# meffmadd/intro-tc-vae

Hardware: AMD Instinct MI355X
Metric: images/sec (64x64x3, z=128, bs=64) intro-TC step (higher is better)
Workload: dtype f32 in/out/accumulate, conv products on split-fp16 MFMA (two scaled fp16 planes, 3 products, fp32-class); 1 GPU; c2: IntroTCSovler.train_step, conv arch, 64x64x3, z_dim=128, channels (64, 128, 256, 512), batch 64/GPU, Adam lr 2e-4, clip 100, N=10000; global_batch=64, parallelism=single, sync_bn=False

## Files before the change

include/itcv_hip.h:

```cpp
#ifndef ITCV_HIP_H
#define ITCV_HIP_H

#include <stddef.h>
#include <stdint.h>

#ifdef __cplusplus
extern "C" {
#endif

#define ITCV_ABI_VERSION 4

int itcv_abi_version(void);
const char* itcv_last_error(void);
int itcv_set_option(const char* name, int value);
int itcv_get_option(const char* name);

int itcv_profile_begin(void);
int itcv_profile_end(void);
int itcv_profile_get(int i, int* code, double* flop, float* ms);
int itcv_profile_clear(void);

size_t itcv_conv2d_packed_weight_elems(int Co, int Ci, int KS, int for_dgrad);
int itcv_conv2d_pack_weight(const float* w, float* wp, int Co, int Ci, int KS, int for_dgrad,
                            void* stream);
// ... 62 lines not shown
int itcv_conv2d_small_cin_bf16x3_supported(int C, int Co, int KS, int W);
int itcv_conv2d_small_cin_fwd_bf16x3(const float* x, const float* w, const float* bias, float* y, int B, int C, int H,
                                     int W, int Co, int KS, int for_dgrad, int ns ,
                                     const float* x_amax , void* stream);
int itcv_conv2d_wgrad_bf16s_supported(int Ci, int H, int W, int Co, int KS);
int itcv_conv2d_wgrad_bf16s(const float* x, const float* dy, float* dw, int B, int Ci, int H, int W, int Co,
                            int KS, int ns, int accumulate, void* ws, size_t ws_bytes, void* stream);
size_t itcv_conv2d_wgrad_workspace(int B, int Ci, int H, int W, int Co, int KS);
int itcv_conv2d_wgrad(const float* x, const float* dy, float* dw, int B, int Ci, int H, int W,
                      int Co, int KS, int up2, int accumulate, void* ws, size_t ws_bytes, void* stream);
int itcv_conv2d_fwd_variant(int B, int Ci, int H, int W, int Co, int KS, int up2);
int itcv_conv2d_wgrad_variant(int B, int Ci, int H, int W, int Co, int KS, int up2);
size_t itcv_bias_grad_workspace(int B, int C, int HW);
int itcv_bias_grad(const float* dy, float* db, int B, int C, int HW, int accumulate, void* ws,
                   size_t ws_bytes, void* stream);

size_t itcv_bn_workspace(int B, int C, int HW);
int itcv_bn_moments(const float* x, double* sums, int B, int C, int HW, void* ws, size_t ws_bytes,
                    void* stream);
int itcv_bn_train_stats(const float* x, int B, int C, int HW, float eps, float momentum, float* running_mean,
                        float* running_var, int64_t* num_batches_tracked, float* mean, float* rstd, void* ws,
                        size_t ws_bytes, void* stream);
int itcv_bn_finalize(const double* sums, double count, float eps, float momentum, float* running_mean,
                     float* running_var, int64_t* num_batches_tracked, float* mean, float* rstd, int C,
                     void* stream);
int itcv_bn_finalize_uv(const double* sums, double count, float eps, float momentum, float* running_mean,
                        float* running_var, int64_t* num_batches_tracked, float* mean, float* rstd, float* unbiased_var,
                        int C, void* stream);
int itcv_bn_eval_stats(const float* running_mean, const float* running_var, float eps, float* mean,
                       float* rstd, int C, void* stream);
// ... 192 lines not shown
                        int loss_type, int reduction, float scale, void* stream);
int itcv_exp_elbo_fwd(const float* a, const float* b, float* out, float* w, int B, float c, void* stream);
int itcv_exp_elbo_bwd(const float* g, const float* w, float* da, float* db, int B, void* stream);
int itcv_lincomb_fwd(const float* const* terms, const float* weights, int n, float* out, void* stream);
int itcv_lincomb_bwd(const float* g, const float* weights, int n, float* grads, void* stream);

size_t itcv_sumsq_workspace(size_t n);
int itcv_sumsq(const float* x, size_t n, double* out, void* ws, size_t ws_bytes, void* stream);
int itcv_clip_coef(const double* sumsq, int nparts, double clip, float* norm_out, float* coef_out,
                   void* stream);
int itcv_scale_by_dev(float* x, size_t n, const float* coef_dev, void* stream);
int itcv_adam_step(float* p, const float* g, float* m, float* v, size_t n, float lr, float beta1,
                   float beta2, float eps, int step, void* stream);
int itcv_adam_step_dev(float* p, const float* g, float* m, float* v, size_t n, float lr, float beta1,
                       float beta2, float eps, int* step_dev, void* stream);
#define ITCV_OPT_MAXIMIZE 0x1
#define ITCV_OPT_NESTEROV 0x2
#define ITCV_OPT_AMSGRAD 0x4
#define ITCV_OPT_DECOUPLED_WD 0x8
#define ITCV_OPT_CENTERED 0x10
int itcv_adamx_step_dev(float* p, const float* g, float* exp_avg, float* exp_avg_sq, float* max_exp_avg_sq,
                        const unsigned char* live, size_t n, double lr, double beta1, double beta2, double eps,
                        double weight_decay, int flags, int* step_dev, void* stream);
int itcv_sgd_step_dev(float* p, const float* g, float* momentum_buffer, const unsigned char* live, size_t n, double lr,
                      double momentum, double dampening, double weight_decay, int flags, int* step_dev, void* stream);
int itcv_adagrad_step_dev(float* p, const float* g, float* sum, const unsigned char* live, size_t n, double lr,
                          double lr_decay, double weight_decay, double eps, int flags, int* step_dev, void* stream);
int itcv_rmsprop_step_dev(float* p, const float* g, float* square_avg, float* momentum_buffer, float* grad_avg,
                          const unsigned char* live, size_t n, double lr, double alpha, double eps,
                          double weight_decay, double momentum, int flags, int* step_dev, void* stream);
// ... 10 lines not shown
```

intro-tc-vae_amd/csrc/conv_igemm.hip:

```cpp
#include "conv_shared.h"

namespace itcv {



constexpr uint32_t kOobBase = 0x80000000u;

__device__ __forceinline__ float buf_load_s(__amdgpu_buffer_rsrc_t r, uint32_t voff, uint32_t soff) {
  return __builtin_bit_cast(float, __builtin_amdgcn_raw_buffer_load_b32(r, voff, __builtin_amdgcn_readfirstlane(soff), 0));
}

__host__ __device__ inline int tile_rows_for(int M) { return M <= 32 ? 32 : (M <= 64 ? 64 : 128); }

struct ConvArgs {
  const float* x;
  const float* wp;
  const float* bias;
  float* y;
  int B, Ci, H, W, Co;
  int Cip, Mp, N;
  int mt, nt;
  int ktiles, ktiles_per_split, cpt;
  uint32_t x_bytes;
  size_t slab_stride;
// ... 1876 lines not shown
  const size_t beg = (size_t)s * chunk, end = beg + chunk < total ? beg + chunk : total;
  double acc = 0.0;
  for (size_t i = beg + threadIdx.x; i < end; i += 256) {
    const size_t b = i / HW, hw = i - b * HW;
    acc += (double)dy[(b * C + c) * HW + hw];
  }
  acc = block_sum(acc, scratch);
  if (threadIdx.x == 0) part[(size_t)s * C + c] = acc;
}
__global__ void bias_grad_combine(const double* __restrict__ part, float* __restrict__ db, int C, int splits,
                                  int accumulate) {
  const int c = blockIdx.x * blockDim.x + threadIdx.x;
  if (c >= C) return;
  const double s = fold_strided(0.0, part + c, (size_t)C, splits);
  db[c] = (accumulate ? db[c] : 0.f) + (float)s;
}

static inline int pad_to(int c, int m) { return (c + m - 1) / m * m; }
static inline int pad16(int c) { return pad_to(c, 16); }
static inline int pad32(int c) { return pad_to(c, 32); }

static int check_ws(const char* name, const void* ws, size_t ws_bytes, size_t need) {
  if (need && (!ws || ws_bytes < need)) return fail("%s: workspace too small (need %lld bytes)", name, (long long)need);
  return 0;
}

static int reduce_fwd_splits(const char* name, const void* ws, const float* bias, float* y, size_t out_elems, int splits,
                             int HW, int Co, hipStream_t st) {
  if (splits <= 1) return 0;
  const int blocks = (int)(cdivz(out_elems, 256) < 2048 ? cdivz(out_elems, 256) : 2048);
// ... 869 lines not shown
}

int itcv_bias_grad(const float* dy, float* db, int B, int C, int HW, int accumulate, void* ws, size_t ws_bytes,
                   void* stream) {
  ITCV_REQUIRE(dy && db && B > 0 && C > 0 && HW > 0, "itcv_bias_grad");
  const int splits = bias_splits(B, C, HW);
  ITCV_REQUIRE(ws && ws_bytes >= (size_t)splits * C * sizeof(double), "itcv_bias_grad(workspace)");
  double* part = static_cast<double*>(ws);
  hipLaunchKernelGGL(bias_grad_partial, dim3(C, splits), dim3(256), 0, S(stream), dy, part, B, C, HW, splits);
  ITCV_CHECK_LAUNCH("itcv_bias_grad");
  hipLaunchKernelGGL(bias_grad_combine, dim3(cdiv(C, 256)), dim3(256), 0, S(stream), part, db, C, splits, accumulate);
  ITCV_CHECK_LAUNCH("itcv_bias_grad(combine)");
  return 0;
}

}
```

intro-tc-vae_amd/csrc/loss_optim.hip:

```cpp
#include <math.h>

#include "common.h"

namespace itcv {

template <int LT>
__device__ __forceinline__ float rec_err(float r, float t) {
  if (LT == ITCV_LOSS_MSE) {
    const float d = r - t;
    return d * d;
  }
  if (LT == ITCV_LOSS_L1) return fabsf(r - t);
  return -(t * fmaxf(logf(r), -100.f) + (1.f - t) * fmaxf(logf(1.f - r), -100.f));
}
template <int LT>
__device__ __forceinline__ float rec_derr(float r, float t) {
  if (LT == ITCV_LOSS_MSE) return 2.f * (r - t);
  if (LT == ITCV_LOSS_L1) return r > t ? 1.f : (r < t ? -1.f : 0.f);
  return (r - t) / fmaxf((1.f - r) * r, 1e-12f);
}

template <int LT>
__global__ __launch_bounds__(256) void recon_partial_kernel(const float* __restrict__ x,
                                                           const float* __restrict__ recon,
// ... 155 lines not shown
                                const int* __restrict__ step_dev) {
  const int step = step_dev[0] + 1;
  const double bc1 = 1.0 - pow((double)b1, (double)step), bc2 = 1.0 - pow((double)b2, (double)step);
  const float step_size = (float)((double)lr / bc1), sqrt_bc2 = (float)sqrt(bc2);
  for (size_t i = (size_t)blockIdx.x * blockDim.x + threadIdx.x; i < n; i += (size_t)gridDim.x * blockDim.x) {
    const float gi = g[i];
    const float mi = m[i] + (1.f - b1) * (gi - m[i]);
    const float vi = b2 * v[i] + (1.f - b2) * gi * gi;
    m[i] = mi;
    v[i] = vi;
    p[i] -= step_size * (mi / (sqrtf(vi) / sqrt_bc2 + eps));
  }
}
__global__ void bump_step_kernel(int* step_dev) { step_dev[0] += 1; }

__global__ void hflip_kernel(const float* __restrict__ x, float* __restrict__ y, const unsigned char* __restrict__ flip,
                             size_t rows_per_image, int W, size_t n) {
  for (size_t i = (size_t)blockIdx.x * blockDim.x + threadIdx.x; i < n; i += (size_t)gridDim.x * blockDim.x) {
    const size_t row = i / W;
    const int w = (int)(i - row * W);
    y[i] = flip[row / rows_per_image] ? x[row * W + (W - 1 - w)] : x[i];
  }
}

__global__ void fill_kernel(float* __restrict__ x, size_t n, float value) {
  for (size_t i = (size_t)blockIdx.x * blockDim.x + threadIdx.x; i < n; i += (size_t)gridDim.x * blockDim.x)
    x[i] = value;
}

constexpr int kSumsqBlocks = 1024;

}

using namespace itcv;

extern "C" {

size_t itcv_recon_workspace(int B, size_t P) {
  return B > 0 && P > 0 ? (size_t)B * recon_splits(B, P) * sizeof(double) : 0;
}

int itcv_recon_rows_fwd(const float* x, const float* recon, float* rows, int B, size_t P, int loss_type, void* ws,
                        size_t ws_bytes, void* stream) {
  ITCV_REQUIRE(x && recon && rows && B > 0 && P > 0, "itcv_recon_rows_fwd");
  const int splits = recon_splits(B, P);
// ... 107 lines not shown
  a.n = n;
  for (int k = 0; k < n; ++k) a.weight[k] = weights[k];
  hipLaunchKernelGGL(lincomb_bwd_kernel, dim3(1), dim3(64), 0, S(stream), g, a, grads);
  ITCV_CHECK_LAUNCH("itcv_lincomb_bwd");
  return 0;
}

size_t itcv_sumsq_workspace(size_t n) {
  (void)n;
  return kSumsqBlocks * sizeof(double);
}

int itcv_sumsq(const float* x, size_t n, double* out, void* ws, size_t ws_bytes, void* stream) {
  ITCV_REQUIRE(x && out && ws && ws_bytes >= kSumsqBlocks * sizeof(double), "itcv_sumsq");
  ITCV_REQUIRE(((uintptr_t)x & 15) == 0, "itcv_sumsq(16-byte aligned input)");
  int blocks = stream_grid(n, 4);
  if (blocks > kSumsqBlocks) blocks = kSumsqBlocks;
  double* part = static_cast<double*>(ws);
  hipLaunchKernelGGL(sumsq_partial_kernel, dim3(blocks), dim3(256), 0, S(stream), x, n, part);
  ITCV_CHECK_LAUNCH("itcv_sumsq");
  hipLaunchKernelGGL(sumsq_final_kernel, dim3(1), dim3(256), 0, S(stream), part, blocks, out);
  ITCV_CHECK_LAUNCH("itcv_sumsq(final)");
  return 0;
}

int itcv_clip_coef(const double* sumsq, int nparts, double clip, float* norm_out, float* coef_out, void* stream) {
  ITCV_REQUIRE(sumsq && nparts > 0 && norm_out && coef_out, "itcv_clip_coef");
  hipLaunchKernelGGL(clip_coef_kernel, dim3(1), dim3(1), 0, S(stream), sumsq, nparts, clip, norm_out, coef_out);
  ITCV_CHECK_LAUNCH("itcv_clip_coef");
  return 0;
}

// ... 18 lines not shown
  return 0;
}

int itcv_adam_step_dev(float* p, const float* g, float* m, float* v, size_t n, float lr, float beta1, float beta2,
                       float eps, int* step_dev, void* stream) {
  ITCV_REQUIRE(p && g && m && v && step_dev, "itcv_adam_step_dev");
  if (!n) return 0;
  hipLaunchKernelGGL(adam_dev_kernel, dim3(stream_grid(n, 1)), dim3(256), 0, S(stream), p, g, m, v, n, lr, beta1, beta2,
                     eps, step_dev);
  ITCV_CHECK_LAUNCH("itcv_adam_step_dev");
  hipLaunchKernelGGL(bump_step_kernel, dim3(1), dim3(1), 0, S(stream), step_dev);
  ITCV_CHECK_LAUNCH("itcv_adam_step_dev(bump)");
  return 0;
}

int itcv_hflip(const float* x, float* y, const unsigned char* flip, int B, int rows_per_image, int W, void* stream) {
  ITCV_REQUIRE(x && y && flip && x != y && B > 0 && rows_per_image > 0 && W > 0, "itcv_hflip");
  const size_t n = (size_t)B * rows_per_image * W;
  hipLaunchKernelGGL(hflip_kernel, dim3(stream_grid(n, 1)), dim3(256), 0, S(stream), x, y, flip, (size_t)rows_per_image, W, n);
  ITCV_CHECK_LAUNCH("itcv_hflip");
  return 0;
}

int itcv_fill(float* x, size_t n, float value, void* stream) {
  ITCV_REQUIRE(x, "itcv_fill");
  if (!n) return 0;
  hipLaunchKernelGGL(fill_kernel, dim3(stream_grid(n, 1)), dim3(256), 0, S(stream), x, n, value);
  ITCV_CHECK_LAUNCH("itcv_fill");
  return 0;
}
// ... 3 lines not shown
```

intro-tc-vae_amd/csrc/norm_act.hip:

```cpp
#include <stdlib.h>

#include <type_traits>

#include "common.h"

namespace itcv {

constexpr int kRedThreads = 256;

__device__ __forceinline__ uint32_t fdiv(uint32_t a, uint32_t d, int sh) { return sh >= 0 ? (a >> sh) : (a / d); }

struct BnGrp {
  size_t xs;
  size_t os;
  size_t dys;
  size_t ps;
  int cs;
  int G;
  int lv0, lvn;
};
__device__ __forceinline__ bool bn_dead(const BnGrp& g, uint32_t group) {
  return g.lvn > 0 && (group < (uint32_t)g.lv0 || group >= (uint32_t)(g.lv0 + g.lvn));
}

// ... 468 lines not shown
  }
  const float* p = dy + (size_t)bc * (4 * H * W) + (size_t)(2 * h) * (2 * W) + 2 * w;
  const float4 a0 = *reinterpret_cast<const float4*>(p), a1 = *reinterpret_cast<const float4*>(p + 4);
  const float4 b0 = *reinterpret_cast<const float4*>(p + 2 * W), b1 = *reinterpret_cast<const float4*>(p + 2 * W + 4);
  return make_float4((a0.x + a0.y) + (b0.x + b0.y), (a0.z + a0.w) + (b0.z + b0.w), (a1.x + a1.y) + (b1.x + b1.y),
                     (a1.z + a1.w) + (b1.z + b1.w));
}

struct BnBwdFinal {
  double* dsums;
  float* dgamma;
  float* dbeta;
  int accumulate;
};

template <int MODE, bool FUSED, bool MX = false>
__global__ __launch_bounds__(kRedThreads) void bn_bwd_partial_v4(
    const float* __restrict__ x, const float* __restrict__ dy, const float* __restrict__ mean,
    const float* __restrict__ rstd, const float* __restrict__ gamma, const float* __restrict__ beta,
    const float* __restrict__ skip, double* __restrict__ part, int B, int C, int H, int W, float slope, int splits,
    int w_shift, int hw_shift, BnBwdFinal f, BnGrp grp, float* __restrict__ mx = nullptr, int nmx = 0) {
  __shared__ double scratch[kRedThreads / 64];
  __shared__ float mscratch[MX ? 2 * (kRedThreads / 64) : 1];
  const uint32_t gz = FUSED ? 0u : blockIdx.z;
  const uint32_t c = blockIdx.x, s = blockIdx.y, HW = H * W, total = (uint32_t)B * HW;
  const uint32_t chunk = ((total + splits - 1) / splits + 3) & ~3u;
  const uint32_t beg = s * chunk, end = min(beg + chunk, total);
  const float ga = gamma[c], be = beta[c];
  const int ngroups = (FUSED && grp.G > 1) ? grp.G : 1;
  if (!FUSED) {
    const size_t g = blockIdx.z;
    x += g * grp.xs, dy += g * grp.dys, mean += g * grp.cs, rstd += g * grp.cs, part += g * splits * 2 * C;
    if (skip) skip += g * grp.xs;
  }
  float acc_db = 0.f, acc_dg = 0.f;
  if (FUSED && threadIdx.x == 0 && f.accumulate) {
    if (f.dbeta) acc_db = f.dbeta[c];
    if (f.dgamma) acc_dg = f.dgamma[c];
  }
 for (int gi = 0; gi < ngroups; ++gi, x += grp.xs, dy += grp.dys, mean += grp.cs, rstd += grp.cs, f.dsums += 2 * grp.cs) {
  if (skip && gi) skip += grp.xs;
  const float mu = mean[c], rs = rstd[c];
  double s1 = 0.0, s2 = 0.0;
  float gmax = 0.f, xmax = 0.f;
  const bool dead = bn_dead(grp, FUSED ? (uint32_t)gi : gz);
  const uint32_t gend = (dead && !MX) ? beg : end;
  constexpr int U = 4;
  for (uint32_t i0 = beg + threadIdx.x * 4; i0 < gend; i0 += kRedThreads * 4 * U) {
    float4 xv4[U], g4[U], k4[U];
    bool ok[U];
#pragma unroll
    for (int u = 0; u < U; ++u) {
      const uint32_t iu = i0 + (uint32_t)u * kRedThreads * 4;
      ok[u] = iu < end;
      const uint32_t i = ok[u] ? iu : i0;
      const uint32_t b = fdiv(i, HW, hw_shift), hw = i - b * HW;
      const uint32_t h = fdiv(hw, W, w_shift), w = hw - h * W;
      const uint32_t bc = b * C + c;
      xv4[u] = *reinterpret_cast<const float4*>(x + (size_t)bc * HW + hw);
      g4[u] = dead ? make_float4(0.f, 0.f, 0.f, 0.f) : upstream4<MODE>(dy, bc, h, w, H, W);
// ... 469 lines not shown
  ITCV_REQUIRE(!p.ws_need || (ws && ws_bytes >= p.ws_need), who);
  ITCV_REQUIRE(!p.f16 || p.vec, "itcv_bn_train_bwd(fp16 planes need W % 4 == 0)");
  double* part = static_cast<double*>(ws);
  float* mx = p.f16 ? reinterpret_cast<float*>(part + p.part_doubles) : nullptr;
  const bool fused = p.vec && p.splits == 1;
  const BnBwdFinal bf = fused ? BnBwdFinal{dsums, dgamma, dbeta, accumulate} : BnBwdFinal{};
  pick<3>(p.mode, [&](auto mode_c) {
    constexpr int MODE = decltype(mode_c)::value;
    if (!p.vec) {
      hipLaunchKernelGGL(bn_bwd_partial<MODE>, p.rgrid, dim3(kRedThreads), 0, st, x, dy, mean, rstd, gamma, beta, skip, part,
                         B, C, H, W, slope, p.splits);
      return;
    }
    pick<2>(fused ? 1 : 0, [&](auto fused_c) {
      pick<2>(p.f16 ? 1 : 0, [&](auto mx_c) {
        hipLaunchKernelGGL((bn_bwd_partial_v4<MODE, decltype(fused_c)::value != 0, decltype(mx_c)::value != 0>), p.rgrid,
                           dim3(kRedThreads), 0, st, x, dy, mean, rstd, gamma, beta, skip, part, B, C, H, W, slope, p.splits,
                           ilog2_exact(W), ilog2_exact(H * W), bf, p.grp, mx, p.nmx);
      });
    });
  });
  ITCV_CHECK_LAUNCH(who);
  if (!fused && p.path != BnPath::SlicedFold) {
    hipLaunchKernelGGL(bn_combine_param_groups_kernel, dim3(cdiv(C, 256)), dim3(256), 0, st, part, dsums, C, p.splits, p.G,
                       dgamma, dbeta, accumulate);
    ITCV_CHECK_LAUNCH(who);
  }
  return 0;
}

static int bn_bwd_apply_launch(const BnPlan& p, const float* x, const float* dy, const float* mean, const float* rstd,
                               const float* gamma, const float* beta, const float* skip, const double* dsums, double count,
                               float* dx, float* dskip, void* dx_planes, int ns, int B, int C, int H, int W, float slope,
// ... 347 lines not shown
```

intro-tc-vae_amd/hipvae/abi.py:

```python
import ctypes
import os
import subprocess

import torch

_HERE = os.path.dirname(os.path.abspath(__file__))
PKG_ROOT = os.path.dirname(_HERE)
LIB_PATH = os.environ.get("ITCV_LIB") or os.path.join(PKG_ROOT, "lib", "libitcv_hip.so")
CSRC = os.path.join(PKG_ROOT, "csrc")
ABI_VERSION = 4

p, i32, i64, sz, f32, f64 = (ctypes.c_void_p, ctypes.c_int, ctypes.c_int64, ctypes.c_size_t,
                             ctypes.c_float, ctypes.c_double)

SIGNATURES = {
    "itcv_abi_version": (i32, []),
    "itcv_last_error": (ctypes.c_char_p, []),
    "itcv_set_option": (i32, [ctypes.c_char_p, i32]),
    "itcv_get_option": (i32, [ctypes.c_char_p]),
    "itcv_profile_begin": (i32, []),
    "itcv_profile_end": (i32, []),
    "itcv_profile_get": (i32, [i32, p, p, p]),
    "itcv_profile_clear": (i32, []),
    "itcv_conv2d_packed_weight_elems": (sz, [i32, i32, i32, i32]),
# ... 36 lines not shown
    "itcv_conv2d_small_cout_bf16p_supported": (i32, [i32, i32, i32]),
    "itcv_conv2d_small_cout_fwd_bf16p": (i32, [p, p, p, p] + [i32] * 8 + [p]),
    "itcv_conv2d_small_cout_fwd": (i32, [p, p, p, p] + [i32] * 7 + [p]),
    "itcv_conv2d_small_cin_supported": (i32, [i32, i32]),
    "itcv_conv2d_small_cin_fwd": (i32, [p, p, p, p] + [i32] * 7 + [p]),
    "itcv_conv2d_small_cin_bf16x3_supported": (i32, [i32, i32, i32, i32]),
    "itcv_conv2d_small_cin_fwd_bf16x3": (i32, [p, p, p, p] + [i32] * 8 + [p, p]),
    "itcv_conv2d_wgrad_bf16s_supported": (i32, [i32] * 5),
    "itcv_conv2d_wgrad_bf16s": (i32, [p, p, p] + [i32] * 8 + [p, sz, p]),
    "itcv_conv2d_wgrad_workspace": (sz, [i32] * 6),
    "itcv_conv2d_wgrad": (i32, [p, p, p, i32, i32, i32, i32, i32, i32, i32, i32, p, sz, p]),
    "itcv_conv2d_fwd_variant": (i32, [i32] * 7),
    "itcv_conv2d_wgrad_variant": (i32, [i32] * 7),
    "itcv_bias_grad_workspace": (sz, [i32, i32, i32]),
    "itcv_bias_grad": (i32, [p, p, i32, i32, i32, i32, p, sz, p]),
    "itcv_bn_workspace": (sz, [i32, i32, i32]),
    "itcv_bn_moments": (i32, [p, p, i32, i32, i32, p, sz, p]),
    "itcv_bn_train_stats": (i32, [p, i32, i32, i32, f32, f32, p, p, p, p, p, p, sz, p]),
    "itcv_bn_finalize": (i32, [p, f64, f32, f32, p, p, p, p, p, i32, p]),
    "itcv_bn_finalize_uv": (i32, [p, f64, f32, f32, p, p, p, p, p, p, i32, p]),
    "itcv_bn_eval_stats": (i32, [p, p, f32, p, p, i32, p]),
    "itcv_bn_act_planes_supported": (i32, [i32] * 4),
    "itcv_bn_act_fwd": (i32, [p, p, p, p, p, p, p, i32, i32, i32, i32, f32, i32, p, i32, sz, p]),
    "itcv_bn_act_bwd_reduce": (i32, [p, p, p, p, p, p, p, p, p, p, i32, i32, i32, i32, i32, f32, i32, i32, p, sz,
                                     p]),
    "itcv_bn_act_bwd_apply": (i32, [p, p, p, p, p, p, p, p, p, f64, p, p, p, p, i32, i32, i32, i32, i32, f32,
                                    i32, i32, p, i32, sz, p]),
    "itcv_bn_train_fwd": (i32, [p, p, p, p, p, p, i32, i32, i32, i32, i32, f32, i32, f32, f32, p, p, p, p, p, p, sz, sz, p, i32, i32,
                                i32, p]),
    "itcv_bn_train_fwd_uv": (i32, [p, p, p, p, p, p, i32, i32, i32, i32, i32, f32, i32, f32, f32, p, p, p, p, p, p, p, sz, sz, p, i32,
# ... 72 lines not shown
    "itcv_recon_workspace": (sz, [i32, sz]),
    "itcv_recon_rows_fwd": (i32, [p, p, p, i32, sz, i32, p, sz, p]),
    "itcv_recon_rows_bwd": (i32, [p, p, p, p, i32, sz, i32, p]),
    "itcv_recon_loss_fwd": (i32, [p, p, p, i32, sz, i32, i32, f32, p, sz, p]),
    "itcv_recon_loss_bwd": (i32, [p, p, p, p, i32, sz, i32, i32, f32, p]),
    "itcv_exp_elbo_fwd": (i32, [p, p, p, p, i32, f32, p]),
    "itcv_exp_elbo_bwd": (i32, [p, p, p, p, i32, p]),
    "itcv_lincomb_fwd": (i32, [p, p, i32, p, p]),
    "itcv_lincomb_bwd": (i32, [p, p, i32, p, p]),
    "itcv_sumsq_workspace": (sz, [sz]),
    "itcv_sumsq": (i32, [p, sz, p, p, sz, p]),
    "itcv_clip_coef": (i32, [p, i32, f64, p, p, p]),
    "itcv_scale_by_dev": (i32, [p, sz, p, p]),
    "itcv_adam_step": (i32, [p, p, p, p, sz, f32, f32, f32, f32, i32, p]),
    "itcv_adam_step_dev": (i32, [p, p, p, p, sz, f32, f32, f32, f32, p, p]),
    "itcv_adamx_step_dev": (i32, [p] * 6 + [sz] + [f64] * 5 + [i32, p, p]),
    "itcv_sgd_step_dev": (i32, [p] * 4 + [sz] + [f64] * 4 + [i32, p, p]),
    "itcv_adagrad_step_dev": (i32, [p] * 4 + [sz] + [f64] * 4 + [i32, p, p]),
    "itcv_rmsprop_step_dev": (i32, [p] * 6 + [sz] + [f64] * 5 + [i32, p, p]),
    "itcv_fill": (i32, [p, sz, f32, p]),
    "itcv_hflip": (i32, [p, p, p, i32, i32, i32, p]),
    "itcv_gather_u8": (i32, [p, i64, i32, i32, p, i32, p, p, p, p]),
}

TC_VAR_FROM_ROW, TC_EPS_DENSITY, TC_WEIGHTED = 1, 2, 4
TC_LIVE = TC_VAR_FROM_ROW | TC_EPS_DENSITY
BN_PATHS = ("OneBlock", "SlicedFold", "SlicedCombine", "Fallback", "PerGroup", "TileStats")
LOSS_TYPES = {"mse": 0, "l1": 1, "bce": 2}
OPT_MAXIMIZE, OPT_NESTEROV, OPT_AMSGRAD, OPT_DECOUPLED_WD, OPT_CENTERED = 0x1, 0x2, 0x4, 0x8, 0x10

# ... 92 lines not shown
```

intro-tc-vae_amd/hipvae/flat.py:

```python
import weakref

import torch

from . import abi
from .abi import call, lib, ptr, stream
from .functional import bump_weight_epoch, register_pack_group

F32 = torch.float32


class FlatGroup:
    def __init__(self, params, inherit=None, grad_free=()):
        self.params = [p for p in params]
        assert self.params, "empty parameter group"
        dev = self.params[0].device
        self.offsets, total = [], 0
        for p in self.params:
            self.offsets.append(total)
            total += (p.numel() + 3) // 4 * 4
        self.numel = total
        self.flat_p = torch.zeros(total, dtype=F32, device=dev)
        self.flat_g = torch.zeros(total, dtype=F32, device=dev)
        self.exp_avg = torch.zeros(total, dtype=F32, device=dev)
        self.exp_avg_sq = torch.zeros(total, dtype=F32, device=dev)
# ... 118 lines not shown
        for p, o in zip(self.params, self.offsets):
            want = self.flat_g.data_ptr() + 4 * o
            if p.grad is None or p.grad.data_ptr() != want:
                p.grad = self.flat_g[o:o + p.numel()].view(p.shape)

    def zero_grad(self):
        call("itcv_fill", ptr(self.flat_g), self.numel, 0.0, stream())
        self.attach_grads()

    def sumsq_into(self, out_f64_slot):
        call("itcv_sumsq", ptr(self.flat_g), self.numel, ptr(out_f64_slot), ptr(self._ws), self._ws.numel(), stream())

    def scale_grads(self, coef_dev):
        call("itcv_scale_by_dev", ptr(self.flat_g), self.numel, ptr(coef_dev), stream())

    def adam_step(self, lr, betas=(0.9, 0.999), eps=1e-8):
        self.step += 1
        call("itcv_adam_step_dev", ptr(self.flat_p), ptr(self.flat_g), ptr(self.exp_avg), ptr(self.exp_avg_sq),
             self.numel, float(lr), float(betas[0]), float(betas[1]), float(eps), ptr(self.step_dev), stream())
        bump_weight_epoch(self.params)

    def fused_step(self, spec):
        kind, flags, hp = spec
        if kind == "adam":
            self.adam_step(*hp)
            return
        self.step += 1
        s, live = self.slots, ptr(self.live)
        head = (ptr(self.flat_p), ptr(self.flat_g))
        if kind == "adamx":
# ... 1 lines not shown
                 live, self.numel, *hp, flags, ptr(self.step_dev), stream())
        elif kind == "sgd":
            call("itcv_sgd_step_dev", *head, ptr(s.get("momentum_buffer")), live, self.numel, *hp, flags,
                 ptr(self.step_dev), stream())
        elif kind == "adagrad":
            call("itcv_adagrad_step_dev", *head, ptr(s["sum"]), live, self.numel, *hp, flags, ptr(self.step_dev),
                 stream())
        elif kind == "rmsprop":
            call("itcv_rmsprop_step_dev", *head, ptr(s["square_avg"]), ptr(s.get("momentum_buffer")),
                 ptr(s.get("grad_avg")), live, self.numel, *hp, flags, ptr(self.step_dev), stream())
        else:
            raise ValueError(f"unknown fused update {kind!r}")
        bump_weight_epoch(self.params)


def clip_grad_norm(groups, clip):
    dev = groups[0].flat_g.device
    sumsq = torch.empty(len(groups), dtype=torch.float64, device=dev)
    for i, g in enumerate(groups):
        g.sumsq_into(sumsq[i:i + 1])
    out = torch.empty(2, dtype=F32, device=dev)
    call("itcv_clip_coef", ptr(sumsq), len(groups), float(clip), ptr(out[0:1]), ptr(out[1:2]), stream())
    for g in groups:
        g.scale_grads(out[1:2])
    return out[0:1]


_NUMBER = (float, int)


def _scalar(v):
    return v.__class__ in _NUMBER or (isinstance(v, (float, int)) and not isinstance(v, bool))


def fused_update(opt):
    t = type(opt)
    keys = _HP_KEYS.get(t)
    if keys is None or len(opt.param_groups) != 1:
        return None
    g = opt.param_groups[0]
# ... 52 lines not shown
```

intro-tc-vae_amd/hipvae/functional.py:

```python
import contextlib
import weakref

import torch
import torch.distributed as dist
from torch.autograd import Function
from torch.autograd.function import once_differentiable

from . import abi
from .abi import call, lib, ptr, stream

F32 = torch.float32


def set_option(name, value):
    call("itcv_set_option", name.encode(), int(value))


def get_option(name):
    return lib.itcv_get_option(name.encode())


@contextlib.contextmanager
def option_scope(name, value):
    prev = get_option(name)
# ... 525 lines not shown
    if ns in (2, 3) and lib.itcv_conv2d_wgrad_bf16s_supported(Ci, H, W, Co, KS):
        if up2:
            xu = torch.empty((B, Ci, H, W), dtype=F32, device=x.device)
            call("itcv_upsample2_fwd", ptr(x), ptr(xu), B * Ci, H // 2, W // 2, stream())
            x = xu

        call("itcv_conv2d_wgrad_bf16s", ptr(x), ptr(dy), ptr(dw), B, Ci, H, W, Co, KS, ns, int(accumulate), ptr(ws), nws,
             stream())
        return dw

    call("itcv_conv2d_wgrad", ptr(x), ptr(dy), ptr(dw), B, Ci, H, W, Co, KS, int(up2), int(accumulate), ptr(ws), nws,
         stream())
    return dw


def bias_grad_raw(dy, B, C, HW, target=None):
    db = target if target is not None else torch.empty((C,), dtype=F32, device=dy.device)
    nws = lib.itcv_bias_grad_workspace(B, C, HW)
    ws = _ws(nws, dy.device)
    call("itcv_bias_grad", ptr(dy), ptr(db), B, C, HW, int(target is not None), ptr(ws), nws, stream())
    return None if target is not None else db


PLANES_STATS = [0, 0]


def _tag_planes(t, planes, ns, fp32_valid=True):
    t._itcv_planes = (planes, ns, t._version, t.data_ptr(), fp32_valid)


def _require_fp32(t, what):
    tag = getattr(t, "_itcv_planes", None)
    if tag is not None and not tag[4]:
        raise abi.HipExtensionError(f"{what}: this tensor was produced as planes only (fp32 values not written)")
    return t
# ... 1225 lines not shown
```

intro-tc-vae_amd/solvers/vae.py:

```python
from typing import Optional

import torch
from torch import Tensor

from hipvae import ddp
from hipvae.functional import LinCombFn, conv_math_scope, deferred_wgrad_reduces, direct_grad_accumulation
from hipvae.flat import FlatGroup, clip_grad_norm, fused_update
from models import grad_free_parameters
from ops import kl_divergence, reconstruction_loss
from utils import SingletonWriter

try:
    from dataset import DisentanglementDataset
except Exception:
    class DisentanglementDataset:
        pass


class VAESolver:
    def __init__(self, dataset, model, batch_size: int, optimizer_e, optimizer_d, recon_loss_type: str,
                 beta_kl: float, beta_rec: float, device: torch.device, use_amp: bool, grad_scaler,
                 writer=None, test_iter: int = 1000, clip: Optional[float] = None):
        self.dataset = dataset
        if isinstance(dataset, DisentanglementDataset):
# ... 77 lines not shown
        groups = [self._group(p) for p in parts]
        for g in groups:
            g.zero_grad()
        with direct_grad_accumulation(), deferred_wgrad_reduces():
            loss.backward(retain_graph=retain_graph, inputs=inputs)
        if defer_average:
            pending = [ddp.average_async(g.flat_g) for g in groups]
            return lambda: [f() for f in pending]
        for g in groups:
            ddp.average_(g.flat_g)
        return None

    def _clip(self):
        if not self.clip:
            return None
        return clip_grad_norm([self._group("encoder"), self._group("decoder")], self.clip)

    def _step(self, part):
        opt = self.optimizer_e if part == "encoder" else self.optimizer_d
        spec = fused_update(opt)
        if spec is None:
            opt.step()
        else:
            g = self._group(part)
            g.bind_optimizer(opt, spec)
            g.fused_step(spec)

    def enable_graph(self, flag: bool = True):
        self._graph_on = bool(flag)
        self._graph = None
        self._graphs, self._graph_warm = {}, {}
        return self

    def _graph_ok(self, specs=None):
        import ops
        if not (getattr(self, "_graph_on", False) and self.writer is None
                and (ddp.get() is None or ddp.graph_capturable())
                and ops._noise["queue"] is None and ops._noise["mode"] == "device"):
            return False
        if specs is None:
# ... 172 lines not shown
```

Before: 4269 images/s.

## Fuse grad-clip norm with Adam step and single-launch bias grad

```diff
diff --git a/include/itcv_hip.h b/include/itcv_hip.h
--- a/include/itcv_hip.h
+++ b/include/itcv_hip.h
@@ -100,6 +100,9 @@
 size_t itcv_bias_grad_workspace(int B, int C, int HW);
 int itcv_bias_grad(const float* dy, float* db, int B, int C, int HW, int accumulate, void* ws,
                    size_t ws_bytes, void* stream);
+int itcv_bias_grad_one_launch(int B, int C, int HW);
+int itcv_bias_grad_fused(const float* dy, float* db, int B, int C, int HW, int accumulate, int two_launches, void* ws,
+                         size_t ws_bytes, void* stream);
 
 size_t itcv_bn_workspace(int B, int C, int HW);
 int itcv_bn_moments(const float* x, double* sums, int B, int C, int HW, void* ws, size_t ws_bytes,
@@ -322,6 +325,14 @@
                    float beta2, float eps, int step, void* stream);
 int itcv_adam_step_dev(float* p, const float* g, float* m, float* v, size_t n, float lr, float beta1,
                        float beta2, float eps, int* step_dev, void* stream);
+#define ITCV_CLIP_MAX_GROUPS 8
+size_t itcv_clip_groups_workspace(int groups);
+int itcv_clip_groups_blocks(size_t n);
+int itcv_clip_groups(const float* const* g, const size_t* n, int* const* step_dev, int groups, double clip,
+                     float* norm_out, float* coef_out, void* ws, size_t ws_bytes, void* stream);
+int itcv_adam_step_clip_dev(float* p, float* g, float* m, float* v, size_t n, float lr, float beta1, float beta2,
+                            float eps, const int* step_dev, const float* coef_dev, float* const* other,
+                            const size_t* other_n, int others, void* stream);
 #define ITCV_OPT_MAXIMIZE 0x1
 #define ITCV_OPT_NESTEROV 0x2
 #define ITCV_OPT_AMSGRAD 0x4
diff --git a/intro-tc-vae_amd/csrc/conv_igemm.hip b/intro-tc-vae_amd/csrc/conv_igemm.hip
--- a/intro-tc-vae_amd/csrc/conv_igemm.hip
+++ b/intro-tc-vae_amd/csrc/conv_igemm.hip
@@ -1914,6 +1914,22 @@
   if (c >= C) return;
   const double s = fold_strided(0.0, part + c, (size_t)C, splits);
   db[c] = (accumulate ? db[c] : 0.f) + (float)s;
+}
+__global__ __launch_bounds__(256) void bias_grad_one(const float* __restrict__ dy, float* __restrict__ db, int B, int C,
+                                                     int HW, int accumulate) {
+  __shared__ double scratch[4];
+  const int c = blockIdx.x;
+  const size_t total = (size_t)B * HW;
+  double acc = 0.0;
+  for (size_t i = threadIdx.x; i < total; i += 256) {
+    const size_t b = i / HW, hw = i - b * HW;
+    acc += (double)dy[(b * C + c) * HW + hw];
+  }
+  acc = block_sum(acc, scratch);
+  if (threadIdx.x == 0) {
+    const double s = 0.0 + acc;
+    db[c] = (accumulate ? db[c] : 0.f) + (float)s;
+  }
 }
 
 static inline int pad_to(int c, int m) { return (c + m - 1) / m * m; }
@@ -2813,4 +2829,18 @@
   return 0;
 }
 
-}
+int itcv_bias_grad_one_launch(int B, int C, int HW) {
+  return B > 0 && C > 0 && HW > 0 && bias_splits(B, C, HW) == 1 ? 1 : 0;
+}
+
+int itcv_bias_grad_fused(const float* dy, float* db, int B, int C, int HW, int accumulate, int two_launches, void* ws,
+                         size_t ws_bytes, void* stream) {
+  ITCV_REQUIRE(dy && db && B > 0 && C > 0 && HW > 0, "itcv_bias_grad_fused");
+  if (two_launches || !itcv_bias_grad_one_launch(B, C, HW))
+    return itcv_bias_grad(dy, db, B, C, HW, accumulate, ws, ws_bytes, stream);
+  hipLaunchKernelGGL(bias_grad_one, dim3(C), dim3(256), 0, S(stream), dy, db, B, C, HW, accumulate);
+  ITCV_CHECK_LAUNCH("itcv_bias_grad_fused");
+  return 0;
+}
+
+}
diff --git a/intro-tc-vae_amd/csrc/loss_optim.hip b/intro-tc-vae_amd/csrc/loss_optim.hip
--- a/intro-tc-vae_amd/csrc/loss_optim.hip
+++ b/intro-tc-vae_amd/csrc/loss_optim.hip
@@ -193,6 +193,104 @@
 }
 __global__ void bump_step_kernel(int* step_dev) { step_dev[0] += 1; }
 
+constexpr int kSumsqBlocks = 1024;
+constexpr int kClipGroups = ITCV_CLIP_MAX_GROUPS;
+static inline int sumsq_blocks(size_t n) {
+  const int b = stream_grid(n, 4);
+  return b > kSumsqBlocks ? kSumsqBlocks : b;
+}
+struct ClipGroups {
+  const float* g[kClipGroups];
+  size_t n[kClipGroups];
+  int first[kClipGroups + 1];
+  int* step[kClipGroups];
+  int groups;
+};
+__global__ __launch_bounds__(256) void clip_partial_kernel(ClipGroups a, double* __restrict__ part) {
+  __shared__ double scratch[4];
+  int k = 0;
+  while (k + 1 < a.groups && (int)blockIdx.x >= a.first[k + 1]) ++k;
+  const uint32_t blk = blockIdx.x - a.first[k], nblk = a.first[k + 1] - a.first[k];
+  const float* __restrict__ x = a.g[k];
+  const size_t n = a.n[k], n4 = n / 4;
+  double acc = 0.0;
+  for (size_t i = (size_t)blk * 256 + threadIdx.x; i < n4; i += (size_t)nblk * 256) {
+    const float4 v = reinterpret_cast<const float4*>(x)[i];
+    acc += (double)v.x * v.x + (double)v.y * v.y + (double)v.z * v.z + (double)v.w * v.w;
+  }
+  if (blk == 0)
+    for (size_t i = n4 * 4 + threadIdx.x; i < n; i += 256) acc += (double)x[i] * x[i];
+  acc = block_sum(acc, scratch);
+  if (threadIdx.x == 0) part[(size_t)k * kSumsqBlocks + blk] = acc;
+}
+__global__ __launch_bounds__(256) void clip_final_kernel(ClipGroups a, const double* __restrict__ part, double clip,
+                                                        float* __restrict__ norm_out, float* __restrict__ coef_out) {
+  __shared__ double scratch[4];
+  double s = 0.0;
+  for (int k = 0; k < a.groups; ++k) {
+    const int nparts = a.first[k + 1] - a.first[k];
+    double acc = 0.0;
+    for (int i = threadIdx.x; i < nparts; i += 256) acc += part[(size_t)k * kSumsqBlocks + i];
+    s += block_sum(acc, scratch);
+  }
+  if (threadIdx.x) return;
+  const double total = sqrt(s);
+  double coef = clip / (total + 1e-6);
+  if (coef > 1.0) coef = 1.0;
+  norm_out[0] = (float)total;
+  coef_out[0] = (float)coef;
+  for (int k = 0; k < a.groups; ++k)
+    if (a.step[k]) a.step[k][0] += 1;
+}
+
+__device__ __forceinline__ float scaled_grad(float x, float c) {
+  float r = x * c;
+  asm volatile("" : "+v"(r));
+  return r;
+}
+struct ScaleGroups {
+  float* x[kClipGroups];
+  size_t n[kClipGroups];
+  int first[kClipGroups + 1];
+  int groups;
+};
+__global__ __launch_bounds__(256) void adam_clip_dev_kernel(float* __restrict__ p, float* __restrict__ g,
+                                                           float* __restrict__ m, float* __restrict__ v, size_t n,
+                                                           float lr, float b1, float b2, float eps,
+                                                           const int* __restrict__ step_dev,
+                                                           const float* __restrict__ coef, int adam_blocks,
+                                                           ScaleGroups o) {
+  const float c = coef[0];
+  if ((int)blockIdx.x >= adam_blocks) {
+    int k = 0;
+    const int rel = (int)blockIdx.x - adam_blocks;
+    while (k + 1 < o.groups && rel >= o.first[k + 1]) ++k;
+    const uint32_t blk = rel - o.first[k], nblk = o.first[k + 1] - o.first[k];
+    float* __restrict__ x = o.x[k];
+    const size_t nk = o.n[k], n4 = nk / 4;
+    for (size_t i = (size_t)blk * 256 + threadIdx.x; i < n4; i += (size_t)nblk * 256) {
+      float4 q = reinterpret_cast<float4*>(x)[i];
+      q.x *= c, q.y *= c, q.z *= c, q.w *= c;
+      reinterpret_cast<float4*>(x)[i] = q;
+    }
+    if (blk == 0)
+      for (size_t i = n4 * 4 + threadIdx.x; i < nk; i += 256) x[i] *= c;
+    return;
+  }
+  const int step = step_dev[0];
+  const double bc1 = 1.0 - pow((double)b1, (double)step), bc2 = 1.0 - pow((double)b2, (double)step);
+  const float step_size = (float)((double)lr / bc1), sqrt_bc2 = (float)sqrt(bc2);
+  for (size_t i = (size_t)blockIdx.x * 256 + threadIdx.x; i < n; i += (size_t)adam_blocks * 256) {
+    const float gi = scaled_grad(g[i], c);
+    g[i] = gi;
+    const float mi = m[i] + (1.f - b1) * (gi - m[i]);
+    const float vi = b2 * v[i] + (1.f - b2) * gi * gi;
+    m[i] = mi;
+    v[i] = vi;
+    p[i] -= step_size * (mi / (sqrtf(vi) / sqrt_bc2 + eps));
+  }
+}
+
 __global__ void hflip_kernel(const float* __restrict__ x, float* __restrict__ y, const unsigned char* __restrict__ flip,
                              size_t rows_per_image, int W, size_t n) {
   for (size_t i = (size_t)blockIdx.x * blockDim.x + threadIdx.x; i < n; i += (size_t)gridDim.x * blockDim.x) {
@@ -206,8 +304,6 @@
   for (size_t i = (size_t)blockIdx.x * blockDim.x + threadIdx.x; i < n; i += (size_t)gridDim.x * blockDim.x)
     x[i] = value;
 }
-
-constexpr int kSumsqBlocks = 1024;
 
 }
 
@@ -345,8 +441,7 @@
 int itcv_sumsq(const float* x, size_t n, double* out, void* ws, size_t ws_bytes, void* stream) {
   ITCV_REQUIRE(x && out && ws && ws_bytes >= kSumsqBlocks * sizeof(double), "itcv_sumsq");
   ITCV_REQUIRE(((uintptr_t)x & 15) == 0, "itcv_sumsq(16-byte aligned input)");
-  int blocks = stream_grid(n, 4);
-  if (blocks > kSumsqBlocks) blocks = kSumsqBlocks;
+  const int blocks = sumsq_blocks(n);
   double* part = static_cast<double*>(ws);
   hipLaunchKernelGGL(sumsq_partial_kernel, dim3(blocks), dim3(256), 0, S(stream), x, n, part);
   ITCV_CHECK_LAUNCH("itcv_sumsq");
@@ -395,6 +490,55 @@
   return 0;
 }
 
+size_t itcv_clip_groups_workspace(int groups) {
+  return groups > 0 && groups <= kClipGroups ? (size_t)groups * kSumsqBlocks * sizeof(double) : 0;
+}
+
+int itcv_clip_groups_blocks(size_t n) { return sumsq_blocks(n); }
+
+int itcv_clip_groups(const float* const* g, const size_t* n, int* const* step_dev, int groups, double clip,
+                     float* norm_out, float* coef_out, void* ws, size_t ws_bytes, void* stream) {
+  ITCV_REQUIRE(g && n && norm_out && coef_out, "itcv_clip_groups");
+  ITCV_REQUIRE(groups >= 1 && groups <= kClipGroups, "itcv_clip_groups(1 .. ITCV_CLIP_MAX_GROUPS groups)");
+  ITCV_REQUIRE(ws && ws_bytes >= (size_t)groups * kSumsqBlocks * sizeof(double), "itcv_clip_groups(workspace)");
+  ClipGroups a;
+  memset(&a, 0, sizeof(a));
+  a.groups = groups;
+  for (int k = 0; k < groups; ++k) {
+    ITCV_REQUIRE(g[k] && ((uintptr_t)g[k] & 15) == 0, "itcv_clip_groups(16-byte aligned group)");
+    a.g[k] = g[k], a.n[k] = n[k], a.step[k] = step_dev ? step_dev[k] : nullptr;
+    a.first[k + 1] = a.first[k] + sumsq_blocks(n[k]);
+  }
+  double* part = static_cast<double*>(ws);
+  hipLaunchKernelGGL(clip_partial_kernel, dim3(a.first[groups]), dim3(256), 0, S(stream), a, part);
+  ITCV_CHECK_LAUNCH("itcv_clip_groups");
+  hipLaunchKernelGGL(clip_final_kernel, dim3(1), dim3(256), 0, S(stream), a, part, clip, norm_out, coef_out);
+  ITCV_CHECK_LAUNCH("itcv_clip_groups(final)");
+  return 0;
+}
+
+int itcv_adam_step_clip_dev(float* p, float* g, float* m, float* v, size_t n, float lr, float beta1, float beta2,
+                            float eps, const int* step_dev, const float* coef_dev, float* const* other,
+                            const size_t* other_n, int others, void* stream) {
+  ITCV_REQUIRE(p && g && m && v && step_dev && coef_dev && n > 0, "itcv_adam_step_clip_dev");
+  ITCV_REQUIRE(others >= 0 && others <= kClipGroups && (!others || (other && other_n)),
+               "itcv_adam_step_clip_dev(0 .. ITCV_CLIP_MAX_GROUPS other groups)");
+  ScaleGroups o;
+  memset(&o, 0, sizeof(o));
+  for (int k = 0; k < others; ++k) {
+    ITCV_REQUIRE(other[k] && ((uintptr_t)other[k] & 15) == 0, "itcv_adam_step_clip_dev(16-byte aligned group)");
+    if (!other_n[k]) continue;
+    const int j = o.groups++;
+    o.x[j] = other[k], o.n[j] = other_n[k];
+    o.first[j + 1] = o.first[j] + stream_grid(other_n[k], 4);
+  }
+  const int adam_blocks = stream_grid(n, 1);
+  hipLaunchKernelGGL(adam_clip_dev_kernel, dim3(adam_blocks + o.first[o.groups]), dim3(256), 0, S(stream), p, g, m, v, n,
+                     lr, beta1, beta2, eps, step_dev, coef_dev, adam_blocks, o);
+  ITCV_CHECK_LAUNCH("itcv_adam_step_clip_dev");
+  return 0;
+}
+
 int itcv_hflip(const float* x, float* y, const unsigned char* flip, int B, int rows_per_image, int W, void* stream) {
   ITCV_REQUIRE(x && y && flip && x != y && B > 0 && rows_per_image > 0 && W > 0, "itcv_hflip");
   const size_t n = (size_t)B * rows_per_image * W;
diff --git a/intro-tc-vae_amd/csrc/norm_act.hip b/intro-tc-vae_amd/csrc/norm_act.hip
--- a/intro-tc-vae_amd/csrc/norm_act.hip
+++ b/intro-tc-vae_amd/csrc/norm_act.hip
@@ -506,7 +506,7 @@
   int accumulate;
 };
 
-template <int MODE, bool FUSED, bool MX = false>
+template <int MODE, bool FUSED, bool MX = false, bool LIVE = false>
 __global__ __launch_bounds__(kRedThreads) void bn_bwd_partial_v4(
     const float* __restrict__ x, const float* __restrict__ dy, const float* __restrict__ mean,
     const float* __restrict__ rstd, const float* __restrict__ gamma, const float* __restrict__ beta,
@@ -535,7 +535,7 @@
   const float mu = mean[c], rs = rstd[c];
   double s1 = 0.0, s2 = 0.0;
   float gmax = 0.f, xmax = 0.f;
-  const bool dead = bn_dead(grp, FUSED ? (uint32_t)gi : gz);
+  const bool dead = LIVE && bn_dead(grp, FUSED ? (uint32_t)gi : gz);
   const uint32_t gend = (dead && !MX) ? beg : end;
   constexpr int U = 4;
   for (uint32_t i0 = beg + threadIdx.x * 4; i0 < gend; i0 += kRedThreads * 4 * U) {
@@ -1035,9 +1035,12 @@
     }
     pick<2>(fused ? 1 : 0, [&](auto fused_c) {
       pick<2>(p.f16 ? 1 : 0, [&](auto mx_c) {
-        hipLaunchKernelGGL((bn_bwd_partial_v4<MODE, decltype(fused_c)::value != 0, decltype(mx_c)::value != 0>), p.rgrid,
-                           dim3(kRedThreads), 0, st, x, dy, mean, rstd, gamma, beta, skip, part, B, C, H, W, slope, p.splits,
-                           ilog2_exact(W), ilog2_exact(H * W), bf, p.grp, mx, p.nmx);
+        pick<2>(p.grp.lvn > 0 ? 1 : 0, [&](auto live_c) {
+          hipLaunchKernelGGL((bn_bwd_partial_v4<MODE, decltype(fused_c)::value != 0, decltype(mx_c)::value != 0,
+                                                decltype(live_c)::value != 0>),
+                             p.rgrid, dim3(kRedThreads), 0, st, x, dy, mean, rstd, gamma, beta, skip, part, B, C, H, W, slope,
+                             p.splits, ilog2_exact(W), ilog2_exact(H * W), bf, p.grp, mx, p.nmx);
+        });
       });
     });
   });
diff --git a/intro-tc-vae_amd/hipvae/abi.py b/intro-tc-vae_amd/hipvae/abi.py
--- a/intro-tc-vae_amd/hipvae/abi.py
+++ b/intro-tc-vae_amd/hipvae/abi.py
@@ -74,6 +74,8 @@
     "itcv_conv2d_wgrad_variant": (i32, [i32] * 7),
     "itcv_bias_grad_workspace": (sz, [i32, i32, i32]),
     "itcv_bias_grad": (i32, [p, p, i32, i32, i32, i32, p, sz, p]),
+    "itcv_bias_grad_one_launch": (i32, [i32, i32, i32]),
+    "itcv_bias_grad_fused": (i32, [p, p, i32, i32, i32, i32, i32, p, sz, p]),
     "itcv_bn_workspace": (sz, [i32, i32, i32]),
     "itcv_bn_moments": (i32, [p, p, i32, i32, i32, p, sz, p]),
     "itcv_bn_train_stats": (i32, [p, i32, i32, i32, f32, f32, p, p, p, p, p, p, sz, p]),
@@ -176,6 +178,10 @@
     "itcv_scale_by_dev": (i32, [p, sz, p, p]),
     "itcv_adam_step": (i32, [p, p, p, p, sz, f32, f32, f32, f32, i32, p]),
     "itcv_adam_step_dev": (i32, [p, p, p, p, sz, f32, f32, f32, f32, p, p]),
+    "itcv_clip_groups_workspace": (sz, [i32]),
+    "itcv_clip_groups_blocks": (i32, [sz]),
+    "itcv_clip_groups": (i32, [p, p, p, i32, f64, p, p, p, sz, p]),
+    "itcv_adam_step_clip_dev": (i32, [p, p, p, p, sz, f32, f32, f32, f32, p, p, p, p, i32, p]),
     "itcv_adamx_step_dev": (i32, [p] * 6 + [sz] + [f64] * 5 + [i32, p, p]),
     "itcv_sgd_step_dev": (i32, [p] * 4 + [sz] + [f64] * 4 + [i32, p, p]),
     "itcv_adagrad_step_dev": (i32, [p] * 4 + [sz] + [f64] * 4 + [i32, p, p]),
diff --git a/intro-tc-vae_amd/hipvae/flat.py b/intro-tc-vae_amd/hipvae/flat.py
--- a/intro-tc-vae_amd/hipvae/flat.py
+++ b/intro-tc-vae_amd/hipvae/flat.py
@@ -1,3 +1,4 @@
+import ctypes
 import weakref
 
 import torch
@@ -156,6 +157,13 @@
     def scale_grads(self, coef_dev):
         call("itcv_scale_by_dev", ptr(self.flat_g), self.numel, ptr(coef_dev), stream())
 
+    def _clip_workspace(self, k):
+        ws = self.__dict__.get("_clip_ws")
+        need = lib.itcv_clip_groups_workspace(k)
+        if ws is None or ws.numel() < need:
+            ws = self._clip_ws = torch.empty(need, dtype=torch.uint8, device=self.flat_g.device)
+        return ws
+
     def adam_step(self, lr, betas=(0.9, 0.999), eps=1e-8):
         self.step += 1
         call("itcv_adam_step_dev", ptr(self.flat_p), ptr(self.flat_g), ptr(self.exp_avg), ptr(self.exp_avg_sq),
@@ -187,16 +195,47 @@
         bump_weight_epoch(self.params)
 
 
-def clip_grad_norm(groups, clip):
+def clip_grad_norm(groups, clip, out=None):
     dev = groups[0].flat_g.device
     sumsq = torch.empty(len(groups), dtype=torch.float64, device=dev)
     for i, g in enumerate(groups):
         g.sumsq_into(sumsq[i:i + 1])
-    out = torch.empty(2, dtype=F32, device=dev)
+    if out is None:
+        out = torch.empty(2, dtype=F32, device=dev)
     call("itcv_clip_coef", ptr(sumsq), len(groups), float(clip), ptr(out[0:1]), ptr(out[1:2]), stream())
     for g in groups:
         g.scale_grads(out[1:2])
     return out[0:1]
+
+
+FUSED_STEP_TAIL = True
+
+
+class DeferredClip:
+
+    def __init__(self, groups, clip):
+        self.groups, self.clip = list(groups), float(clip)
+        self.out = torch.empty(2, dtype=F32, device=groups[0].flat_g.device)
+        self.norm = self.out[0:1]
+
+    def run(self):
+        clip_grad_norm(self.groups, self.clip, out=self.out)
+
+    def run_with_adam(self, trained, lr, betas=(0.9, 0.999), eps=1e-8):
+        groups, k = self.groups, len(self.groups)
+        assert any(g is trained for g in groups), "the updated group is not among the clipped ones"
+        vp, szt = ctypes.c_void_p, ctypes.c_size_t
+        ws = trained._clip_workspace(k)
+        call("itcv_clip_groups", (vp * k)(*[g.flat_g.data_ptr() for g in groups]), (szt * k)(*[g.numel for g in groups]),
+             (vp * k)(*[g.step_dev.data_ptr() if g is trained else None for g in groups]), k, self.clip,
+             ptr(self.out[0:1]), ptr(self.out[1:2]), ptr(ws), ws.numel(), stream())
+        rest = [g for g in groups if g is not trained]
+        trained.step += 1
+        call("itcv_adam_step_clip_dev", ptr(trained.flat_p), ptr(trained.flat_g), ptr(trained.exp_avg),
+             ptr(trained.exp_avg_sq), trained.numel, float(lr), float(betas[0]), float(betas[1]), float(eps),
+             ptr(trained.step_dev), ptr(self.out[1:2]), (vp * len(rest))(*[g.flat_g.data_ptr() for g in rest]),
+             (szt * len(rest))(*[g.numel for g in rest]), len(rest), stream())
+        bump_weight_epoch(trained.params)
 
 
 _NUMBER = (float, int)
diff --git a/intro-tc-vae_amd/hipvae/functional.py b/intro-tc-vae_amd/hipvae/functional.py
--- a/intro-tc-vae_amd/hipvae/functional.py
+++ b/intro-tc-vae_amd/hipvae/functional.py
@@ -563,11 +563,15 @@
     return dw
 
 
+BIAS_GRAD_ONE_LAUNCH = True
+
+
 def bias_grad_raw(dy, B, C, HW, target=None):
     db = target if target is not None else torch.empty((C,), dtype=F32, device=dy.device)
     nws = lib.itcv_bias_grad_workspace(B, C, HW)
     ws = _ws(nws, dy.device)
-    call("itcv_bias_grad", ptr(dy), ptr(db), B, C, HW, int(target is not None), ptr(ws), nws, stream())
+    call("itcv_bias_grad_fused", ptr(dy), ptr(db), B, C, HW, int(target is not None), int(not BIAS_GRAD_ONE_LAUNCH),
+         ptr(ws), nws, stream())
     return None if target is not None else db
 
 
diff --git a/intro-tc-vae_amd/solvers/vae.py b/intro-tc-vae_amd/solvers/vae.py
--- a/intro-tc-vae_amd/solvers/vae.py
+++ b/intro-tc-vae_amd/solvers/vae.py
@@ -5,6 +5,7 @@
 
 from hipvae import ddp
 from hipvae.functional import LinCombFn, conv_math_scope, deferred_wgrad_reduces, direct_grad_accumulation
+from hipvae import flat
 from hipvae.flat import FlatGroup, clip_grad_norm, fused_update
 from models import grad_free_parameters
 from ops import kl_divergence, reconstruction_loss
@@ -115,16 +116,33 @@
     def _clip(self):
         if not self.clip:
             return None
-        return clip_grad_norm([self._group("encoder"), self._group("decoder")], self.clip)
+        groups = [self._group("encoder"), self._group("decoder")]
+        if not flat.FUSED_STEP_TAIL:
+            return clip_grad_norm(groups, self.clip)
+        self._issue_clip()
+        self._pending_clip = flat.DeferredClip(groups, self.clip)
+        return self._pending_clip.norm
+
+    def _issue_clip(self):
+        pend, self._pending_clip = getattr(self, "_pending_clip", None), None
+        if pend is not None:
+            pend.run()
 
     def _step(self, part):
         opt = self.optimizer_e if part == "encoder" else self.optimizer_d
         spec = fused_update(opt)
         if spec is None:
+            self._issue_clip()
             opt.step()
+            return
+        g = self._group(part)
+        g.bind_optimizer(opt, spec)
+        pend = getattr(self, "_pending_clip", None)
+        if pend is not None and spec[0] == "adam" and any(c is g for c in pend.groups):
+            self._pending_clip = None
+            pend.run_with_adam(g, *spec[2])
         else:
-            g = self._group(part)
-            g.bind_optimizer(opt, spec)
+            self._issue_clip()
             g.fused_step(spec)
 
     def enable_graph(self, flag: bool = True):
```

Measured after the change: 4297 images/s (median of 6 runs). No clear change (+0.6%).
